# fritzsedlazeck/Sniffles

Measured on AMD Instinct MI355X. Metric: SV-signatures clustered/sec (clustering + calling + QC + genotype + INS consensus), higher is better.
Workload: dtype int32/f64

## Files before the change

### include/sniffles_amd.h

```cpp
#ifndef SNIFFLES_AMD_H
#define SNIFFLES_AMD_H

#include <stdint.h>

#ifdef __cplusplus
extern "C" {
#endif

#define SNF_ABI_VERSION 5

#define SNF_SVLEN_NONE INT32_MIN
#define SNF_SEQ_NONE (-1)
#define SNF_PS_NONE (-1)

enum snf_svtype {
  SNF_INS = 0, SNF_DEL = 1, SNF_DUP = 2, SNF_INV = 3, SNF_BND = 4,
  SNF_SINGLE_LEFT = 5, SNF_SINGLE_RIGHT = 6, SNF_NTYPES = 7
};

enum snf_source { SNF_SRC_INLINE = 0, SNF_SRC_SPLIT_PRIM = 1, SNF_SRC_SPLIT_SUP = 2, SNF_SRC_BND_SA = 3 };

enum snf_filter {
  SNF_F_PASS = 0, SNF_F_STDEV_POS, SNF_F_STDEV_LEN, SNF_F_SINGLE_BREAK, SNF_F_SVLEN_MIN,
  SNF_F_STRAND_BND, SNF_F_COV_CHANGE_DEL, SNF_F_COV_CHANGE_DUP, SNF_F_COV_CHANGE_INS,
// ... 219 lines not shown
struct snf_extract;
int snf_batch_add_task_device(snf_batch_t* b, struct snf_extract* x, const snf_task_input_t* meta);
int snf_batch_upload(snf_batch_t* b);
#define SNF_RUN_NONE 0
#define SNF_RUN_CANDIDATES 1
#define SNF_RUN_PASS 0x100
int snf_batch_open(const snf_config_t* cfg, int device, const snf_task_input_t* tasks, int32_t n_tasks, int run, snf_batch_t** out);
void snf_batch_destroy(snf_batch_t* b);

int snf_batch_call_candidates(snf_batch_t* b);

int snf_batch_finalize(snf_batch_t* b);

int snf_batch_pass(snf_batch_t* batch);

enum snf_output { SNF_OUT_CANDIDATES = 0, SNF_OUT_EXECUTE = 1, SNF_OUT_DEVICE = 2 };
int snf_batch_set_output(snf_batch_t* b, int mode);

int snf_batch_set_result_memory(snf_batch_t* b, void* block, int64_t block_bytes, void* alt, int64_t alt_bytes);

int snf_batch_fetch(snf_batch_t* b, int stage, snf_result_t* out);
int64_t snf_batch_n_candidates(snf_batch_t* b);

typedef struct snf_export_layout {
  int64_t n_calls, rnames_len, alt_pool_len;
  int64_t off_rnames, off_alt, bytes;
} snf_export_layout_t;
int snf_batch_export_device(snf_batch_t* b, void* dst_device, int64_t cap_bytes, snf_export_layout_t* layout);

int snf_batch_block_coverage(snf_batch_t* b, int32_t task_index, int32_t binsize, int64_t first_bin,
                             int64_t n_bins, int32_t* out);
// ... 418 lines not shown
```

### sniffles_amd/abi.py

```python
from __future__ import annotations

import ctypes as C
import math

import numpy as np

from .soa import LEAD_FIELDS, TaskInput

ABI_VERSION = 5

FILTERS = [
    "PASS", "STDEV_POS", "STDEV_LEN", "SINGLE_BREAK", "SVLEN_MIN", "STRAND_BND", "COV_CHANGE_DEL",
    "COV_CHANGE_DUP", "COV_CHANGE_INS", "INLINE_SA", "COV_VAR", "COV_CHANGE_FRAC_US", "COV_CHANGE_FRAC_SC",
    "COV_CHANGE_FRAC_CE", "COV_CHANGE_FRAC_ED", "SUPPORT_MIN", "GT_FAILED", "GT", "COV_MIN_GT", "ALN_NM",
    "MOSAIC_VAF", "SVLEN_MAX_MOSAIC", "STRAND", "STRAND_MOSAIC", "SVLEN_MIN_MOSAIC", "COV_MIN",
    "NOT_MOSAIC_VAF", "MOSAIC_SV_CLOSE_EDGE",
]
TASK_OK, TASK_ERR_UNBOUND_END = 0, 1

i32, i64, f64, u8p = C.c_int32, C.c_int64, C.c_double, C.POINTER(C.c_uint8)


class snf_config_t(C.Structure):
    _fields_ = [
# ... 72 lines not shown

class snf_result_t(C.Structure):
    _fields_ = [
        ("n_calls", i64), ("calls", C.POINTER(snf_call_t)),
        ("alt_pool_len", i64), ("alt_pool", u8p),
        ("rnames_len", i64), ("rnames", C.POINTER(C.c_uint32)),
        ("n_tasks", i64), ("task_status", C.POINTER(C.c_int32)),
        ("task_call_off", C.POINTER(C.c_int64)), ("coverage_average_total", C.POINTER(C.c_double)),
    ]


class snf_export_layout_t(C.Structure):
    _fields_ = [("n_calls", i64), ("rnames_len", i64), ("alt_pool_len", i64), ("off_rnames", i64), ("off_alt", i64), ("bytes", i64)]


OUT_CANDIDATES, OUT_EXECUTE, OUT_DEVICE = 0, 1, 2


class snf_clusters_t(C.Structure):
    _fields_ = [("n_clusters", i64)] + [(n, C.POINTER(C.c_int32)) for n in
                                        ("task_index", "svtype", "start", "end", "seed", "seed_index", "n_leads_long")] + \
               [("repeat", u8p), ("lead_off", C.POINTER(C.c_int64)), ("n_leads", i64), ("lead", C.POINTER(C.c_int32)),
                ("lead_svlen", C.POINTER(C.c_int32))]


class snf_combine_problem_t(C.Structure):
    _fields_ = [
        ("svtype", i32), ("n_cands", i32), ("n_groups", i32), ("n_sample_ids", i32),
        ("pos", C.POINTER(C.c_int32)), ("svlen", C.POINTER(C.c_int32)), ("support", C.POINTER(C.c_int32)),
        ("sample_id", C.POINTER(C.c_int32)), ("mate_contig", C.POINTER(C.c_int32)), ("mate_ref_start", C.POINTER(C.c_int32)),
        ("alt_off", C.POINTER(C.c_int64)), ("alt_pool", u8p),
# ... 425 lines not shown
```

### sniffles_amd/csrc/snf_lib.hip

```cpp
#include "snf_stage_final.h"
#include "snf_wave_refine.h"
#include "snf_wave_cons.h"
#include "snf_fused.h"
#include "snf_stage_window.h"
#include "snf_stage_out.h"
#include "snf_wave_call.h"
#include "snf_wave_call_g.h"
#include "snf_wave_refine_g.h"
#include "snf_ctx.h"
#include "snf_genotype.h"

#include <rocprim/device/device_radix_sort.hpp>
#include <rocprim/device/device_scan.hpp>

#include <fcntl.h>
#include <sys/file.h>
#include <unistd.h>

#include <atomic>
#include <map>
#include <tuple>
#include <cmath>
#include <ctime>
#include <memory>
// ... 228 lines not shown
  bool timing = true;
  bool time_all = false;
  int time_every = 8;
  bool time_now = true;
  uint64_t pass_count = 0;
  bool res_current = false;
  int64_t* h_rn_total = nullptr;
  int slots_d1w = 8192, slots_d2w = 8192, slots_e1w = 8192, slots_big = 8192;
  int read_key_bits = 64;
  std::vector<int32_t> h_rend_max;
  bool uploaded = false;
  bool finalized = false;
  int finalize_runs = 0;
  int rn_state = 0;
  int64_t pf_words = 0;
  struct PassGraph { hipGraph_t graph = nullptr; hipGraphExec_t exec = nullptr; int passes = 0; int rn_state = 0; int rn_defer = 0; size_t cap_out = 0, cap_alt = 0; };
  std::map<std::tuple<void*, void*, int>, PassGraph> graphs;
  int graph_mode = 0;
  bool in_flight = false;
  bool side_open = false;
  int slot_fd = -1;
  double pass_start_ms = 0.0;
  bool capturing = false;
  bool staged = false; bool staged_kernel = false, stage_block_copied = false, stage_alt_copied = false;
  bool graph_failed = false;
  int64_t h_n_big64 = 0;
  int64_t h_n_occ = 0; int win_cap = 0;
  bool reads_ready = false;
  bool cov_avg_ready = false;
  double gt_last_ms = 0;
  std::vector<snf_task_input_t> tasks;
// ... 7 lines not shown
  uint8_t* slab = nullptr; size_t slab_cap = 0, slab_used = 0, slab_next = (size_t)64 << 20;
  View v{};
  ReadPrep rp{};
  Counts* h_cnt = nullptr;
  void* sort_tmp[2] = {nullptr, nullptr}; size_t sort_tmp_bytes[2] = {0, 0};
  hipEvent_t ev_cls_fork = nullptr, ev_cls_join = nullptr;
  hipEvent_t ev_refined = nullptr, ev_fcopy = nullptr;
  bool fcopy_open = false;
  hipEvent_t ev_fork = nullptr, ev_join = nullptr, ev_fork3 = nullptr, ev_join3 = nullptr, ev_base = nullptr,
             ev_counts = nullptr, ev_rn = nullptr, ev_join4 = nullptr, ev_e3 = nullptr;
  int64_t tab_cap = 0, aln_cap = 0, cr_cap = 0, alt_cap = 0;
  HostBuf hb_calls, hb_rn, hb_res;
  bool pass_idle = false;
  HostBuf hb_out, hb_alt;
  std::vector<std::pair<void*, size_t>> ext_ranges;
  bool have_hist = false; int64_t hist_calls = 0, hist_small = 0, hist_large = 0, hist_copy = 0;
  bool have_big_hist = false; int64_t hist_big[3] = {0, 0, 0};
  bool skipped_big[3] = {false, false, false};
  int out_mode = 0;
  std::vector<int32_t> r_status; std::vector<int64_t> r_off; std::vector<double> r_cov;
  std::vector<int32_t> cl_task, cl_svtype, cl_start, cl_end, cl_seed, cl_seed_index, cl_nlong, cl_lead, cl_lead_svlen; std::vector<uint8_t> cl_repeat;
  std::vector<int64_t> cl_lead_off;
  std::vector<Timing> timings;
  std::vector<Timing> timing_acc;
  struct Ev { hipEvent_t a, b; const char* name; int64_t bytes; };
  std::vector<Ev> evs; size_t ev_used = 0;
};

template <class T>
T* dalloc_own(snf_batch_impl* b, size_t n) {
  size_t bytes = (n ? n : 1) * sizeof(T);
  void* p = nullptr;
  if (hipMalloc(&p, bytes) != hipSuccess) {
    (void)hipGetLastError();
    p = nullptr;
    g_slabs.trim(b->device);
    SNF_HIP(hipMalloc(&p, bytes));
  }
  b->bufs.push_back({p, bytes});
  return (T*)p;
}
template <class T>
// ... 986 lines not shown
  View& v = b->v;
  const int64_t N = v.NS;
  const dim3 grid(b->slots_d1w);
  const auto d1w = v.fuse_defer ? d1w_refine<true> : d1w_refine<false>;
  if (v.wave_path && b->k.d1_groups) {
    { ClassFork _f(b);
      KERNEL_GRID((v.fuse_defer ? d1g_refine<8, true> : d1g_refine<8, false>), grid, dim3(64), v, 0, "d1g_refine8", N * 36 / 3, heavy); }
    v.d1_from_list = 1;
    KERNEL_GRID(d1w, grid, dim3(64), v, 0, "d1w_refine", N * 36 - N * 36 / 3, heavy);
    v.d1_from_list = 0;
    join_classes(b);
  } else if (v.wave_path)
    KERNEL_GRID(d1w, grid, dim3(64), v, 0, "d1w_refine", N * 36, heavy);
  if (!(v.wave_path && b->fused)) KERNEL_N(d1_refine, v, N, v.wave_path ? 0 : N * 36, quiet);
  b->skipped_big[0] = b->skipped_big[1] = b->skipped_big[2] = false;
  if (v.wave_path && b->have_big_hist && b->hist_big[0] == 0) b->skipped_big[0] = true;
  else if (v.wave_path) KERNEL_GRID(x_big<0>, dim3(b->slots_big), dim3(64), v, 0, "x_big_refine", 0, heavy);
}
void enqueue_call(snf_batch_impl* b) {
  View& v = b->v;
  const int64_t N = v.NS;
  const bool ph = b->cfg.phase != 0;
  const dim3 grid(b->slots_d2w);
  const auto d2w = ph ? d2w_call<5, true> : d2w_call<5, false>;
  if (b->fused && v.chain_on) KERNEL_N(d1bc_rctable, v, N, 0, quiet);
  else if (b->fused) KERNEL_N(d1bk_rctable, v, N, 0, quiet);
  else {
    prim_exscan<uint32_t>(b, v.rcflag, v.rcscan, N + 1, "scan_refined");
    KERNEL_N(d1b_rctable, v, N, N * 4, quiet);
  }
  const bool call_forks = v.wave_path && b->k.d2_groups && classes_beside(b);
  if (v.fuse_defer && !call_forks) enqueue_fuse_copy(b, nullptr);
  if (v.wave_path && b->k.d2_groups) {
    { ClassFork _f(b);
      KERNEL_GRID((ph ? d2g_call<8, 4, true> : d2g_call<8, 4, false>), grid, dim3(64), v, 0, "d2g_call8", N * 32 / 3, heavy); }
    if (v.fuse_defer && call_forks) enqueue_fuse_copy(b, b->ev_cls_fork);
    const bool mid = b->k.d2_mid;
    if (mid) KERNEL_GRID((ph ? d2g_call<32, 4, true> : d2g_call<32, 4, false>), grid, dim3(64), v, 0, "d2g_call32", 0, heavy);
    v.d2_from_list = mid ? 2 : 1;
    KERNEL_GRID(d2w, grid, dim3(64), v, 0, "d2w_call", N * 32 - N * 32 / 3, heavy);
    v.d2_from_list = 0;
    join_classes(b);
  } else if (v.wave_path)
    KERNEL_GRID(d2w, grid, dim3(64), v, 0, "d2w_call", N * 32, heavy);
  if (!(v.wave_path && b->fused)) KERNEL_N(d2_call, v, N, v.wave_path ? 0 : N * 32, quiet);
  if (v.wave_path && b->have_big_hist && b->hist_big[1] == 0) b->skipped_big[1] = true;
  else if (v.wave_path) KERNEL_GRID(x_big<1>, dim3(b->slots_big), dim3(64), v, 0, "x_big_call", 0, heavy);
  if (b->fused && v.chain_on) KERNEL_N(d3cc_compact, v, N, 0, quiet);
  else if (b->fused) KERNEL_N(d3ck_compact, v, N, 0, quiet);
  else {
    prim_exscan<uint32_t>(b, v.cdflag, v.cdscan, N + 1, "scan_calls");
    KERNEL_N(d3_compact, v, N, 0, quiet);
  }
}
void enqueue_candidate_tail(snf_batch_impl* b) {
  View& v = b->v;
  const int64_t N = v.NS;
  KERNEL_N(d3_taskoff, v, tail_threads(v), 0, quiet);
  SNF_HIP(hipEventRecord(b->ev_counts, b->stream));
  fork_mark(b);
  if (b->fused) {
// ... 213 lines not shown
    const int stage_env = b->k.stage_out;
    const bool stage = !(v.out_mode & SNF_OUT_DEVICE) && !b->capturing && (stage_env == 1 || (stage_env < 0 && passes_overlap(b)));
    b->staged = stage; b->staged_kernel = stage && b->k.stage_copy_kernel;
    b->stage_block_copied = b->stage_alt_copied = false;
    const bool out_hbm = (v.out_mode & SNF_OUT_DEVICE) || stage;
    v.out_pin = out_hbm ? nullptr : (uint8_t*)b->hb_out.p;
    v.out_pin_cap = out_hbm ? 0 : (int64_t)b->hb_out.cap;
    v.stage_out_pin = b->staged_kernel ? (uint8_t*)b->hb_out.p : nullptr; v.stage_out_cap = b->staged_kernel ? (int64_t)b->hb_out.cap : 0;
    const size_t want_alt = (size_t)(v.pool_len / 8) + ((size_t)1 << 20);
    if (!(v.out_mode & SNF_OUT_DEVICE) && !b->hb_alt.external && b->hb_alt.cap < want_alt) b->hb_alt.ensure(want_alt);
    v.alt_pin = out_hbm ? nullptr : (uint8_t*)b->hb_alt.p;
    v.alt_pin_cap = out_hbm ? 0 : (int64_t)b->hb_alt.cap;
    v.stage_alt_pin = b->staged_kernel ? (uint8_t*)b->hb_alt.p : nullptr; v.stage_alt_cap = b->staged_kernel ? (int64_t)b->hb_alt.cap : 0;
  }
  v.out_valid = 1;
  int64_t n_calls_hint = b->hist_calls;
  if (!b->have_hist && NS > 0) {
    SNF_HIP(hipEventSynchronize(b->ev_counts));
    n_calls_hint = b->h_cnt->n_calls;
  }
  if (NS > 0) {
  {
    SideStream side(b);
    if (v.wave_path && b->finalize_runs++ > 0) dzero(b, v.big_cnt + 2 * 64 * 16, sizeof(uint32_t) * 64 * 16);
    if (v.wave_path) {
      int64_t grid = (n_calls_hint + v.e1_batch - 1) / v.e1_batch + 1;
      if (grid > (1 << 20)) grid = 1 << 20;
      KERNEL_GRID(e1w_finalize<5>, dim3((unsigned)grid), dim3(64), v, 0, "e1w_finalize", 0, heavy);
    }
    if (!v.wave_path) KERNEL_N(e1_finalize, v, NS, 0, quiet);
    if (v.wave_path && b->have_big_hist && b->hist_big[2] == 0 && b->finalize_runs == 1) b->skipped_big[2] = true;
    else if (v.wave_path) KERNEL_GRID(x_big<2>, dim3(b->slots_big), dim3(64), v, 0, "x_big_finalize", 0, heavy);
  }
  const bool fast_alt = v.wave_path && b->fused && NS <= ((int64_t)1 << 22) * 256;
  if (fast_alt)
  {
    const unsigned grid = (unsigned)((NS + 255) / 256);
    KERNEL_GRID(e2a_sizes, dim3(grid), dim3(256), v, 0, "e2a_sizes", 0, quiet);
    KERNEL_GRID(e3b_offsets, dim3(grid), dim3(256), v, 0, "e3b_offsets", 0, quiet);
    SNF_HIP(hipEventRecord(b->ev_e3, b->stream));
    {
      SideStream side(b);
      SNF_HIP(hipStreamWaitEvent(b->stream2, b->ev_e3, 0));
      SNF_HIP(hipStreamWaitEvent(b->stream2, b->ev_rn, 0));
      enqueue_output_head(b);
      stage_copy_block(b);
    }
    if (!b->have_hist) {
      d2h(b, b->h_cnt, v.cnt, sizeof(Counts));
      dsync(b);
      const Counts& c = *b->h_cnt;
      b->hist_small = (int64_t)c.n_cls[1]; b->hist_large = (int64_t)(c.n_cls[2] + c.n_cls[3] + c.n_cls[4] + c.n_cls[5]); b->hist_copy = (int64_t)c.n_cls[0];
      b->hist_calls = c.n_calls; b->have_hist = true;
    }
    join_fuse_copy(b);
    enqueue_consensus_wave(b, b->hist_small + 1, b->hist_large + 1, b->hist_copy + 1);
    stage_copy_alt(b);
    join_side(b);
    join_fourth(b);
  }
  else
  {
    d2h(b, b->h_cnt, v.cnt, sizeof(Counts));
    dsync(b);
    const int64_t nc = b->h_cnt->n_calls;
    dzero(b, v.stripes, sizeof(unsigned long long) * 4 * 64 * 16);
    KERNEL_N(e2_best, v, nc + 1, 0, heavy);
    prim_exscan<uint32_t>(b, v.fN, v.pN, nc + 1, "scan_alt");
    prim_exscan<uint32_t>(b, v.fL, v.pL, nc + 1, "scan_cons");
    prim_exscan<int64_t>(b, v.sz_tab, v.sc_tab, nc + 1, "scan_cons_sizes");
    prim_exscan<int64_t>(b, v.sz_aln, v.sc_aln, nc + 1, "scan_cons_sizes");
// ... 11 lines not shown
    join_fourth(b);
    enqueue_output_head(b);
  }
  } else {
    join_side(b);
    join_fourth(b);
    enqueue_output_head(b);
  }
  KERNEL_N(z1_results, v, tail_threads(v), 0, quiet);
  b->res_current = true;
}

bool pass_graph_ok(snf_batch_impl* b) {
  const View& v = b->v;
  if (b->graph_mode == 1 && pacing_of(b).passes_in_flight.load() > 1) return false;
  return b->graph_mode && !b->graph_failed && b->have_hist && b->fused && v.front && v.wave_path && !b->k.timeline && !b->time_all &&
         v.NS > 0 && !b->k.readprep_each_pass && !b->k.serial;
}
void run_pass(snf_batch_impl* b) {
  View& v = b->v;
  pass_begins(b);
  join_open_candidates(b);
  if (!pass_graph_ok(b)) { run_call_candidates(b); run_finalize(b); return; }
  const auto key = std::make_tuple((void*)b->hb_out.p, (void*)b->hb_alt.p, v.out_mode);
  auto& g = b->graphs[key];
  if (g.exec && (g.cap_out != b->hb_out.cap || g.cap_alt != b->hb_alt.cap)) {
    (void)hipGraphExecDestroy(g.exec); (void)hipGraphDestroy(g.graph); g = snf_batch_impl::PassGraph{};
  }
  g.passes++;
  const bool sampled = b->timing && (b->time_all || b->time_every == 1 || (b->time_every > 1 && b->pass_count % (uint64_t)b->time_every == 0));
  if (g.exec && !sampled) {
    b->pass_idle = false;
    reset_timing(b); b->pass_count++;
    SNF_HIP(hipGraphLaunch(g.exec, b->stream));
    b->reads_ready = true; b->cov_avg_ready = true; b->finalized = true; b->finalize_runs = 1; b->res_current = true;
    b->rn_state = g.rn_state; v.rn_defer = g.rn_defer; v.out_valid = 1;
    return;
  }
  if (g.exec || g.passes < 2) { run_call_candidates(b); run_finalize(b); return; }
  const bool tm = b->timing;
  b->timing = false;
  hipGraph_t graph = nullptr;
  bool ok = hipStreamBeginCapture(b->stream, hipStreamCaptureModeThreadLocal) == hipSuccess;
  if (ok) {
    b->capturing = true;
    const uint64_t count_before = b->pass_count;
    try { run_call_candidates(b); run_finalize(b); }
    catch (const std::exception& e) {
      (void)hipStreamEndCapture(b->stream, &graph); if (graph) (void)hipGraphDestroy(graph); graph = nullptr; ok = false; (void)hipGetLastError();
      b->pass_count = count_before;
      if (v.prof) fprintf(stderr, "[SNF_PROF] pass graph: capture gave up (%s); the pass runs eagerly\n", e.what());
// ... 5 lines not shown
    b->capturing = false;
    if (ok) ok = hipStreamEndCapture(b->stream, &graph) == hipSuccess && graph != nullptr;
  }
  b->timing = tm;
  hipGraphExec_t exec = nullptr;
  if (ok) ok = hipGraphInstantiate(&exec, graph, nullptr, nullptr, 0) == hipSuccess && exec != nullptr;
  if (!ok) {
    (void)hipGetLastError();
    if (graph) (void)hipGraphDestroy(graph);
    b->graph_failed = true;
    if (v.prof) fprintf(stderr, "[SNF_PROF] pass graph: capture failed, passes stay eager\n");
    run_call_candidates(b); run_finalize(b);
    return;
  }
  g.graph = graph; g.exec = exec; g.rn_state = b->rn_state; g.rn_defer = v.rn_defer; g.cap_out = b->hb_out.cap; g.cap_alt = b->hb_alt.cap;
  if (v.prof) { size_t nn = 0; (void)hipGraphGetNodes(graph, nullptr, &nn); fprintf(stderr, "[SNF_PROF] pass graph: captured (%zu nodes)\n", nn); }
  SNF_HIP(hipGraphLaunch(g.exec, b->stream));
}
void destroy_graphs(snf_batch_impl* b) {
  for (auto& kv : b->graphs) { if (kv.second.exec) (void)hipGraphExecDestroy(kv.second.exec); if (kv.second.graph) (void)hipGraphDestroy(kv.second.graph); }
  b->graphs.clear();
}

void collect_timings(snf_batch_impl* b) {
  b->timings.clear();
#ifdef SNF_ITRACE
  if (b->k.prof && b->v.itrace) {
    static const char* nm[SNF_IT_SLOTS] = {"w1_hist", "w3_scatter", "w4s_segment", "w6t_emit", "d1g_refine", "d1w_refine", "d2g_call", "d2w_call", "e3b_offsets",
                                           "e1w_finalize", "cons SMALL", "cons LARGE", "d4s_coverage", "f4w_emit", "cons ROWS", ""};
    std::vector<uint32_t> h((size_t)SNF_IT_SLOTS * SNF_IT_CAP * 2);
// ... 119 lines not shown

void do_fetch(snf_batch_impl* b, int stage, snf_result_t* out) {
  SNF_TRACE(stage >= 1 ? "snf_batch_fetch(1): wait + result block" : "snf_batch_fetch(0): wait + candidates");
  View& v = b->v;
  int T = v.T;
  b->r_status.assign(T, 0); b->r_off.assign(T + 1, 0); b->r_cov.assign(T, NAN);
  full_sync(b);
  pass_waited(b);
  if (b->h_cnt->overflow) fail(b->h_cnt->overflow & 2 ? "internal: hand-over list of the call kernels overflowed" : "internal: fused-sequence pool overflow");
  if (v.prof) {
    const Counts& c = *b->h_cnt;
    fprintf(stderr, "[SNF_PROF] counts: valid %lld windows %lld bins %lld seeds %lld clusters %lld refined %lld calls %lld | cons calls %lld reads %lld "
                    "fallback %lld alt bytes %lld fused bytes through the shared counter %llu (the rest in the waves' own slices; the split depends on scheduling, the total and the capacity do not) | ALT lists copy %llu small %llu large %llu/%llu/%llu/%llu thread %llu rows %llu\n", (long long)c.n_valid, (long long)c.n_occ, (long long)c.n_bins, (long long)c.n_seeds, (long long)c.n_clusters,
            (long long)c.n_rc, (long long)c.n_calls, (long long)c.n_cons, (long long)c.n_cons_reads, (long long)c.n_cons_fallback,
            (long long)c.alt_total, c.pool_extra_used, c.n_cls[0], c.n_cls[1], c.n_cls[2], c.n_cls[3], c.n_cls[4], c.n_cls[5], c.n_cls[6], c.n_cls[7]);
    fprintf(stderr, "[SNF_PROF] merge scan: %lld runs, %lld groups redone serially (run_gap %d)\n", (long long)c.n_runs, (long long)c.n_dirty_groups, (int)v.run_gap);
  }
  memcpy(b->r_status.data(), v.res_status, (size_t)T * sizeof(int32_t));
  memcpy(b->r_cov.data(), v.res_cov, (size_t)T * sizeof(double));
  if (stage >= 1 && b->finalized) {
    const bool alt_late = settle_alt_stage(b);
    {
      const Counts& c = *b->h_cnt;
      bool skipped_work = false;
      for (int k = 0; k < 3; k++) {
        if (b->skipped_big[k] && c.n_big[k] > 0) skipped_work = true;
        b->hist_big[k] = c.n_big[k];
      }
      if (skipped_work) { b->pass_idle = true; fail("internal: a pass skipped x_big although items were handed to it (the handle's next pass launches it)"); }
      b->have_big_hist = true;
      b->hist_small = (int64_t)c.n_cls[1]; b->hist_large = (int64_t)(c.n_cls[2] + c.n_cls[3] + c.n_cls[4] + c.n_cls[5]); b->hist_copy = (int64_t)c.n_cls[0];
      b->hist_calls = c.n_calls; b->have_hist = true;
    }
    const OutHdr h = *v.res_out;
    const uint8_t* base = (const uint8_t*)b->hb_out.p;
    const int64_t alt_total_now = b->h_cnt->alt_total;
    const bool block_there = !h.in_pinned && b->staged_kernel && b->stage_block_copied && v.stage_out_pin == (uint8_t*)b->hb_out.p && h.bytes <= v.stage_out_cap;
    const bool alt_there = !b->h_cnt->alt_in_pinned && b->staged_kernel && b->stage_alt_copied && !alt_late && v.stage_alt_pin == (uint8_t*)b->hb_alt.p && alt_total_now <= v.stage_alt_cap;
    bool need_sync = false;
    std::unique_lock<std::mutex> copy_turn(pacing_of(b).copy_mu, std::defer_lock);
    if (b->staged && pace_copy_turn() && ((!h.in_pinned && !block_there) || (!b->h_cnt->alt_in_pinned && !alt_there))) copy_turn.lock();
    if (!h.in_pinned && !block_there) {
      v.out_pin = nullptr; v.out_pin_cap = 0;
      base = (const uint8_t*)b->hb_out.ensure((size_t)h.bytes + 256);
      d2h_timed(b, (void*)base, v.out_dev, (size_t)h.bytes, "d2h_block");
      need_sync = true;
    }
// ... 597 lines not shown
}

int snf_batch_upload(snf_batch_t* bb) {
  SNF_TRY({
    auto b = reinterpret_cast<snf_batch_impl*>(bb);
    if (!b) fail("null batch");
    if (b->uploaded) fail("batch already uploaded");
    SNF_HIP(hipSetDevice(b->device));
    do_upload(b);
  })
}

int snf_batch_open(const snf_config_t* cfg, int device, const snf_task_input_t* tasks, int32_t n_tasks, int run, snf_batch_t** out) {
  if (out) *out = nullptr;
  if (!out || (n_tasks > 0 && !tasks) || n_tasks < 0) { g_err = "snf_batch_open: null argument"; return 1; }
  if (run != SNF_RUN_NONE && run != SNF_RUN_CANDIDATES && !((run & SNF_RUN_PASS) && (run & ~SNF_RUN_PASS) <= (SNF_OUT_EXECUTE | SNF_OUT_DEVICE))) {
    g_err = "snf_batch_open: unknown run mode"; return 1;
  }
  snf_batch_t* h = nullptr;
  int rc = snf_batch_create(cfg, device, &h);
  for (int32_t t = 0; rc == 0 && t < n_tasks; t++) rc = snf_batch_add_task(h, &tasks[t]);
  if (rc == 0) rc = snf_batch_upload(h);
  if (rc == 0 && run == SNF_RUN_CANDIDATES) rc = snf_batch_call_candidates(h);
  if (rc == 0 && (run & SNF_RUN_PASS)) { rc = snf_batch_set_output(h, run & ~SNF_RUN_PASS); if (rc == 0) rc = snf_batch_pass(h); }
  if (rc != 0) { const std::string keep = g_err; if (h) snf_batch_destroy(h); g_err = keep; return rc; }
  *out = h;
  return 0;
}

void snf_batch_destroy(snf_batch_t* bb) {
  auto b = reinterpret_cast<snf_batch_impl*>(bb);
// ... 23 lines not shown
  for (auto& e : b->ext_ranges) (void)hipHostUnregister(e.first);
  b->ext_ranges.clear();
  if (b->stream) g_streams.give(b->device, b->stream);
  if (b->stream2) g_streams.give(b->device, b->stream2);
  if (b->stream3) g_streams.give(b->device, b->stream3);
  if (b->stream4) g_streams.give(b->device, b->stream4);
  if (b->ev_join4) (void)hipEventDestroy(b->ev_join4);
  delete b;
}

int snf_batch_call_candidates(snf_batch_t* bb) {
  SNF_TRY({
    auto b = reinterpret_cast<snf_batch_impl*>(bb);
    if (!b || !b->uploaded) fail("batch not uploaded");
    SNF_HIP(hipSetDevice(b->device));
    run_call_candidates(b);
  })
}

int snf_batch_pass(snf_batch_t* bb) {
  SNF_TRY({
    auto b = reinterpret_cast<snf_batch_impl*>(bb);
    if (!b || !b->uploaded) fail("batch not uploaded");
    SNF_HIP(hipSetDevice(b->device));
    run_pass(b);
  })
}

int snf_batch_finalize(snf_batch_t* bb) {
  SNF_TRY({
// ... 31 lines not shown
  if (!b || !b->uploaded || !b->h_cnt) return -1;
  return b->v.NS > 0 ? b->h_cnt->n_calls : 0;
}

int64_t snf_trim_caches(int device) {
  int64_t bytes = (int64_t)g_slabs.trim(device);
  bytes += (int64_t)g_pinned.trim();
  (void)g_streams.trim(device);
  return bytes;
}

int snf_batch_set_output(snf_batch_t* bb, int mode) {
  SNF_TRY({
    auto b = reinterpret_cast<snf_batch_impl*>(bb);
    if (!b) fail("null batch");
    if (mode < 0 || mode > (SNF_OUT_EXECUTE | SNF_OUT_DEVICE)) fail("unknown output mode");
    b->out_mode = mode; b->v.out_mode = mode;
  })
}

int snf_batch_set_result_memory(snf_batch_t* bb, void* block, int64_t block_bytes, void* alt, int64_t alt_bytes) {
  SNF_TRY({
    auto b = reinterpret_cast<snf_batch_impl*>(bb);
    if (!b) fail("null batch");
    if ((block == nullptr) != (alt == nullptr) || block_bytes < 0 || alt_bytes < 0) fail("snf_batch_set_result_memory: both sections or none");
    SNF_HIP(hipSetDevice(b->device));
    if (b->uploaded && !b->pass_idle) full_sync(b);
    if (!block) { b->hb_out.release(); b->hb_alt.release(); }
    else { b->hb_out.adopt(block, (size_t)block_bytes, b->ext_ranges); b->hb_alt.adopt(alt, (size_t)alt_bytes, b->ext_ranges); }
  })
}
// ... 119 lines not shown
```

### sniffles_amd/csrc/snf_stage_cluster.h

```cpp
#pragma once
#include "snf_exact.h"
#include "snf_view.h"

namespace snf {

#define SNF_KEY_INVALID (~0ull)
SNF_HD int key_grp(uint64_t key) { return (int)(key >> 32); }
SNF_HD int grp_svtype(int g) { return g & 7; }
SNF_HD int grp_task(int g) { return g >> 3; }

SNF_HD bool lead_is_long(const View& v, uint32_t o) {
  return v.in_svtype[o] == SNF_INS && v.in_svlen[o] == SNF_SVLEN_NONE;
}

SNF_HD int64_t pf_cell(const View& v, int t, int svtype, uint64_t bin) {
  const int64_t c0 = v.t_cell_off[t], nb = (v.t_cell_off[t + 1] - c0) / SNF_NTYPES;
  return c0 + (int64_t)svtype * nb + (int64_t)bin;
}
SNF_HD void a1_keys_body(int64_t i, const View& v) {
  int t = v.lead_task[i];
  int64_t rs = v.in_ref_start[i];
  bool valid = rs >= 0 && rs < v.t_contig_len[t];
  uint64_t bin = valid ? (uint64_t)(rs / v.cfg.cluster_binsize) : 0;
  const int svtype = v.in_svtype[i];
// ... 73 lines not shown
}

SNF_HD void a4_binstats_body(int64_t b, const View& v) {
  if (b >= v.cnt->n_bins) { v.eligflag[b] = 0; return; }
  int32_t lo = v.bin_lo[b], hi = v.bin_lo[b + 1];
  int n_normal = 0;
  uint32_t hc[3] = {0, 0, 0};
  for (int32_t p = lo; p < hi; p++) {
    uint32_t o = v.val_out[p];
    if (p - lo + 1 > v.cfg.consensus_max_reads_bin) v.seqnull[o] = 1;
    uint8_t h = v.in_hap[o];
    if (hc[h] < 65535u) hc[h]++;
    if (!lead_is_long(v, o)) n_normal++;
  }
  for (int h = 0; h < 3; h++) v.bin_hap[3 * b + h] = (uint16_t)hc[h];
  bool el = n_normal >= v.cfg.dev_min_leads_cluster;
  v.bin_elig[b] = el;
  v.eligflag[b] = el ? 1u : 0u;
  int g = key_grp(v.bin_key[b]);
  if (b == 0 || key_grp(v.bin_key[b - 1]) != g) v.grp_first_bin[g] = (int32_t)b;
}

SNF_HD void a5_leadflags_body(int64_t p, const View& v) {
  uint32_t fn = 0, fl = 0;
  if (p < v.cnt->n_valid) {
    uint32_t b = v.headscan[p + 1] - 1;
    if (v.bin_elig[b]) {
      if (lead_is_long(v, v.val_out[p])) fl = 1; else fn = 1;
    }
  }
  v.fN[p] = fn;
  v.fL[p] = fl;
  if (p == 0) { v.fN[v.NS] = 0; v.fL[v.NS] = 0; v.eligflag[v.NS] = 0; }
}
// ... 327 lines not shown
```

### sniffles_amd/csrc/snf_stage_window.h

```cpp
#pragma once
#include "snf_fused.h"
#include "snf_wave_refine.h"

namespace snf {

#define SNF_WIN_MAXCAP 1024

SNF_HD uint32_t win_pack(const View& v, uint32_t bin_low, bool is_long, uint32_t hap) { return bin_low | ((is_long ? 1u : 0u) << 12) | (hap << 13); }
SNF_HD uint32_t win_bin_low(uint32_t a) { return a & 0xfffu; }
SNF_HD bool win_is_long(uint32_t a) { return (a >> 12) & 1u; }
SNF_HD uint32_t win_hap(uint32_t a) { return (a >> 13) & 3u; }
SNF_D bool win_of_lead(const View& v, int64_t i, uint32_t* w, uint32_t* attr) {
  const int t = v.lead_task[i];
  const int64_t rs = v.in_ref_start[i];
  if (rs < 0 || rs >= v.t_contig_len[t]) return false;
  const uint64_t bin = (uint64_t)(rs / v.cfg.cluster_binsize);
  const int svtype = v.in_svtype[i];
  const int64_t w0 = v.t_win_off[t], nwin = (v.t_win_off[t + 1] - w0) / SNF_NTYPES;
  *w = (uint32_t)(w0 + (int64_t)svtype * nwin + (int64_t)(bin >> v.win_bits));
  *attr = win_pack(v, (uint32_t)(bin & ((1u << v.win_bits) - 1u)), svtype == SNF_INS && v.in_svlen[i] == SNF_SVLEN_NONE, v.in_hap[i]);
  return true;
}

SNF_D int win_group(bool valid, uint32_t w, int* count, bool* leader) {
// ... 138 lines not shown
    if (i >= (int64_t)v.cnt->n_w4big) return;
    i = v.w4_list[i];
  }
  const int64_t B0 = 64 * i;
  const int64_t n_valid = v.win_ready ? v.win_n_valid : v.cnt->n_valid;
  uint64_t w0 = 0;
  if (B0 + lane < n_valid) w0 = v.key_in[B0 + lane];
  uint32_t k0 = 0, k1 = 0;
  if (B0 < n_valid) { k0 = v.blk_k0[i]; k1 = B0 + 64 <= n_valid ? v.blk_k0[i + 1] : (uint32_t)(v.win_ready ? v.win_n_occ : v.cnt->n_occ); }
  const int nw = (int)(k1 - k0);
  if (nw <= 0) { if (lane == 0) { v.ws_seeds[i] = 0; v.ws_nf[i] = 0; v.ws_nl[i] = 0; } return; }
  uint4 wr = make_uint4(0, 0, 0, 0);
  if (lane < nw) wr = ((const uint4*)v.wlist)[k0 + lane];
  const int xlo = (int)((int64_t)(uint32_t)__builtin_amdgcn_readfirstlane((int)wr.z) - B0);
  const int xhi = (int)((int64_t)(uint32_t)__builtin_amdgcn_readlane((int)(wr.z + wr.y), nw - 1) - B0);
  if (v.w4_mode == 1 && __shfl(wave_incl_max(lane < nw ? (int)wr.y : 0), 63, 64) > CAP) {
    if (lane == 0) v.w4_list[atomicAdd(&v.cnt->n_w4big, 1ull)] = (int32_t)i;
    return;
  }
  uint64_t wd[E];
  wd[0] = w0;
#pragma unroll
  for (int j = 1; j < E; j++) { const int x = lane + 64 * j; wd[j] = x < xhi ? v.key_in[B0 + x] : 0ull; }
  if (lane < nw) {
    const int t = (int)wr.w;
    const int64_t o0 = v.t_win_off[t], nwin = (v.t_win_off[t + 1] - o0) / SNF_NTYPES, rem = (int64_t)wr.x - o0;
    wS[lane] = (uint32_t)((int64_t)wr.z - B0); wG[lane] = (uint32_t)(t * 8 + (int)(rem / nwin)); wB[lane] = (uint32_t)((rem % nwin) << v.win_bits);
  }
#pragma unroll
  for (int j = 0; j < E; j++) { const int x = lane + 64 * j; if (x < xhi) { sA[x] = 0; sB[x] = 0; widx[x] = 0; } }
  const int nall = __shfl(wave_incl_max(lane < nw ? (int)wr.y : 0), 63, 64);
  for (int p = lane; p < nall + PAD; p += 64) keys[xhi + p] = ~0ull;
  __syncthreads();
  if (lane < nw) widx[wS[lane]] = (uint16_t)(lane + 1);
  __syncthreads();
  uint64_t e[E];
  {
    int carry = 0;
#pragma unroll
    for (int j = 0; j < E; j++) {
      e[j] = 0;
      if (64 * j < xhi) {
        const int x = lane + 64 * j;
// ... 62 lines not shown
  }
  __syncthreads();
  int cs = 0, cf = 0, cl = 0;
  const unsigned long long below = (1ull << lane) - 1ull;
#pragma unroll
  for (int j = 0; j < E; j++) {
    const int x = lane + 64 * j;
    if (64 * j >= xhi) break;
    const bool own = x >= xlo && x < xhi;
    bool f_seed = false, f_norm = false, f_long = false, f_null = false;
    int h = 0, all = 0, with_len = 0;
    if (own) {
      h = hpos[x];
      const uint32_t A = sA[h];
      all = (int)(A & 0xffffu); with_len = (int)(A >> 16);
      const bool elig = with_len >= v.cfg.dev_min_leads_cluster;
      f_norm = elig && !wkey_long(sk[j]); f_long = elig && wkey_long(sk[j]); f_seed = elig && x == h;
      f_null = x - h + 1 > v.cfg.consensus_max_reads_bin;
    }
    const unsigned long long bn = __ballot(f_norm), bl = __ballot(f_long), bs = __ballot(f_seed);
    const uint32_t rn = (uint32_t)(cf + __popcll(bn & below)), rl = (uint32_t)(cl + __popcll(bl & below)), rs = (uint32_t)(cs + __popcll(bs & below));
    if (own) {
      const uint32_t hi = (f_norm ? SNF_WS_NORM : 0u) | (f_long ? SNF_WS_LONG : 0u) | (f_null ? SNF_WS_SEQNULL : 0u) | (f_seed ? SNF_WS_SEED : 0u) |
                          ((f_norm ? rn : rl) << 4) | ((uint32_t)j << 16) | (f_seed ? rs << 21 : 0u);
      v.key_out[B0 + x] = ((uint64_t)hi << 32) | (uint64_t)wkey_index(sk[j]);
      if (f_seed) {
        const uint32_t B = sB[h];
        const int wl = (int)wkey_widx(sk[j]);
        const int64_t start = ((int64_t)wB[wl] + (int64_t)wkey_bin(sk[j])) * v.cfg.cluster_binsize;
        v.whead[B0 + x] = (uint64_t)with_len | ((uint64_t)all << 16) | ((uint64_t)(B & 0xffffu) << 32) | ((uint64_t)(B >> 16) << 48);
        v.whead2[B0 + x] = (uint64_t)(uint32_t)(int32_t)start | ((uint64_t)wG[wl] << 32) | ((uint64_t)(f_norm ? rl : rn) << 52);
// ... 81 lines not shown
```

### sniffles_amd/csrc/snf_view.h

```cpp
#pragma once
#include "../../include/sniffles_amd.h"
#include "snf_rt.h"

namespace snf {

struct Counts {
  int64_t n_valid, n_bins, n_seeds, NF, NLL, n_runs, n_clusters, n_rc, n_calls;
  int64_t n_ins_calls, alt_total, n_cons, tab_total, aln_total, n_cons_reads, rn_total;
  int64_t n_dirty_groups;
  int64_t n_kept;
  int64_t n_big[3];
  int64_t n_occ;
  int64_t max_win;
  int64_t n_big64;
  unsigned long long n_w4big;
  int64_t n_cons_fallback;
  unsigned long long cons_bytes[4];
  unsigned long long n_cls[8];
  unsigned long long pool_extra_used;
#ifdef SNF_CONS_PROFILE
  unsigned long long dbg[32];
#endif
#ifdef SNF_C1_PROFILE
  unsigned long long c1p[16];
#endif
  int32_t overflow;
  int32_t alt_in_pinned;
};

struct GtEntry {
// ... 109 lines not shown
  uint32_t* rflag;

  const int32_t *nm_start, *nm_end;
  const int64_t* t_nm_off;
  const int32_t* t_cov_exact;

  const int32_t* tr_start; const int32_t* tr_end; const int32_t* tr_pmax;

  int32_t prefilter;
  uint32_t* pf_bm;
  const int64_t* t_cell_off;
  uint64_t* pf_key;
  uint32_t *pf_keep, *pf_scan;
  int32_t front;
  int32_t win_bits;
  int64_t NW;
  const int64_t* t_win_off;
  int32_t win_ready;
  int32_t win_stats;
  int64_t win_n_valid, win_n_occ;
  uint32_t *wcnt, *wfill;
  uint32_t* wbase;
  uint32_t* wlist;
  uint32_t* blk_k0;
  uint32_t *ws_seeds, *ws_nf, *ws_nl;
  uint64_t* whead;
  uint64_t* whead2;
  uint64_t *key_in, *key_out; uint32_t *val_in, *val_out;
  int key32, key_bin_bits, key_nbits;
  uint32_t *headflag, *headscan;
// ... 81 lines not shown
  int32_t* cls_list[8];
  uint32_t* big_cnt;
  int32_t* big_list;
  int64_t big_cap;
  int32_t big_wave;
  int32_t e1_batch;
  int32_t* w4_list; int32_t w4_mode, _pad_w4;
  int32_t heavy_n;
  int32_t wave_uniform;
  int32_t* w7;
  const LeadRec* stage_R; int32_t* stage_w; int32_t stage_cap; int32_t _pad_stage;
  uint8_t* aln_kept_w;
  int64_t* crl_off; int32_t* crl_len;
};

#define SNF_IT_SLOTS 16
#define SNF_IT_CAP (1 << 17)
#ifdef SNF_ITRACE
struct ItScope {
  uint32_t* o; unsigned long long t0;
  __device__ ItScope(const View& v, int slot) : o(nullptr), t0(wall_clock64()) {
    if (v.itrace && threadIdx.x == 0 && blockIdx.x < (unsigned)SNF_IT_CAP) o = v.itrace + 2 * ((int64_t)slot * SNF_IT_CAP + blockIdx.x);
  }
  __device__ ~ItScope() { if (o) { o[0] = (uint32_t)t0; o[1] = (uint32_t)(wall_clock64() - t0) | 0x80000000u; } }
};
#define IT_SCOPE(slot) ItScope it_scope_(v, slot);
#else
#define IT_SCOPE(slot)
#endif

// ... 2 lines not shown
```

### sniffles_amd/parallel.py

```python
from __future__ import annotations

import os

from . import lib, sv
from .abi import TASK_ERR_UNBOUND_END

LAZY_CALLS = os.environ.get("SNF_EAGER_CALLS") != "1"


class Task:
    def __init__(self, id, sv_id, contig, start, end, config, assigned_process_id=None, lead_provider=None,
                 tandem_repeats=None, regions=None, device: int = 0):
        self.id, self.sv_id, self.contig, self.start, self.end = id, sv_id, contig, start, end
        self.config = config
        self.assigned_process_id = assigned_process_id
        self.lead_provider = lead_provider
        self.tandem_repeats = tandem_repeats
        self.regions = regions
        self.device = device
        self.coverage_average_total = None
        self._batch = None
        self._ti = None
        self._prep = None
        self._lazy = None
        self._served = False

    def prepare(self, config, execute=None):
        from .abi import OUT_CANDIDATES, OUT_EXECUTE
        if self._prep is not None or self._server() is not None:
            return
        self._release()
        self._ti = self._task_input(config)
        from .soa import DeviceTaskInput
        if isinstance(self._ti, DeviceTaskInput):
            return
        run = lib.Batch.RUN_CANDIDATES if execute is None else (lib.Batch.RUN_PASS | (OUT_EXECUTE if execute else OUT_CANDIDATES))
        self._prep = {"mode": execute, "pending": lib.Batch.open_in_background(config, [self._ti], device=self.device, run=run)}

    def _prepared(self, execute) -> bool:
        box, self._prep = self._prep, None
        if box is None:
            return False
        if box["mode"] != execute:
            box["pending"].discard()
            return False
        self._batch = box["pending"].result()
        self._adopt()
        return True

    def _task_input(self, config):
        lp = self.lead_provider
# ... 93 lines not shown
                                       keep_all=bool(config.no_qc or getattr(config, "snf", None) is not None))
            out = self._lazy.make()
        else:
            out = sv.materialize_candidates(res, self._ti, 0, len(res.calls), svcall_cls, bnd_cls, sv.SVCallPostprocessingInfo, self._batch)
        self.sv_id += len(out)
        self.coverage_average_total = float(res.coverage_average_total[0])
        return out

    def _drop_lazy(self):
        src = getattr(self, "_lazy", None)
        self._lazy = None
        if src is not None:
            src.detach()

    def call_records(self, config, execute: bool = False):
        from .abi import OUT_CANDIDATES, OUT_EXECUTE
        if not self._prepared(bool(execute)):
            self._open(config)
            self._batch.set_output(OUT_EXECUTE if execute else OUT_CANDIDATES)
            self._batch.run_pass()
        res = self._batch.fetch(1, copy=False)
        if int(res.task_status[0]) == TASK_ERR_UNBOUND_END:
            raise UnboundLocalError("local variable 'end' referenced before assignment")
        self._finalized = True
        self.sv_id += int(self._batch.n_candidates())
        self.coverage_average_total = float(res.coverage_average_total[0])
        return res, self._ti

    def finalize_candidates(self, candidates, keep_qc_fails, config) -> list:
        import numpy as np
        if getattr(self, "_served", False):
            if getattr(self, "_finalized", False):
                raise RuntimeError("finalize_candidates needs the candidates of this task's call_candidates")
            candidates = list(candidates)
# ... 345 lines not shown
```

Measured before the change: 3.776 billion.

## Skip single-breakend seeds and windows in execute passes when QC drops them

```diff
diff --git a/include/sniffles_amd.h b/include/sniffles_amd.h
--- a/include/sniffles_amd.h
+++ b/include/sniffles_amd.h
@@ -257,7 +257,7 @@
 
 int snf_batch_pass(snf_batch_t* batch);
 
-enum snf_output { SNF_OUT_CANDIDATES = 0, SNF_OUT_EXECUTE = 1, SNF_OUT_DEVICE = 2 };
+enum snf_output { SNF_OUT_CANDIDATES = 0, SNF_OUT_EXECUTE = 1, SNF_OUT_DEVICE = 2, SNF_OUT_ALL_CANDIDATES = 4 };
 int snf_batch_set_output(snf_batch_t* b, int mode);
 
 int snf_batch_set_result_memory(snf_batch_t* b, void* block, int64_t block_bytes, void* alt, int64_t alt_bytes);
diff --git a/sniffles_amd/abi.py b/sniffles_amd/abi.py
--- a/sniffles_amd/abi.py
+++ b/sniffles_amd/abi.py
@@ -110,7 +110,7 @@
     _fields_ = [("n_calls", i64), ("rnames_len", i64), ("alt_pool_len", i64), ("off_rnames", i64), ("off_alt", i64), ("bytes", i64)]
 
 
-OUT_CANDIDATES, OUT_EXECUTE, OUT_DEVICE = 0, 1, 2
+OUT_CANDIDATES, OUT_EXECUTE, OUT_DEVICE, OUT_ALL_CANDIDATES = 0, 1, 2, 4
 
 
 class snf_clusters_t(C.Structure):
diff --git a/sniffles_amd/csrc/snf_lib.hip b/sniffles_amd/csrc/snf_lib.hip
--- a/sniffles_amd/csrc/snf_lib.hip
+++ b/sniffles_amd/csrc/snf_lib.hip
@@ -266,7 +266,8 @@
   int finalize_runs = 0;
   int rn_state = 0;
   int64_t pf_words = 0;
-  struct PassGraph { hipGraph_t graph = nullptr; hipGraphExec_t exec = nullptr; int passes = 0; int rn_state = 0; int rn_defer = 0; size_t cap_out = 0, cap_alt = 0; };
+  struct PassGraph { hipGraph_t graph = nullptr; hipGraphExec_t exec = nullptr; int passes = 0; int rn_state = 0; int rn_defer = 0; size_t cap_out = 0, cap_alt = 0;
+                     bool skipped_big[3] = {false, false, false}; };
   std::map<std::tuple<void*, void*, int>, PassGraph> graphs;
   int graph_mode = 0;
   bool in_flight = false;
@@ -304,8 +305,10 @@
   bool pass_idle = false;
   HostBuf hb_out, hb_alt;
   std::vector<std::pair<void*, size_t>> ext_ranges;
-  bool have_hist = false; int64_t hist_calls = 0, hist_small = 0, hist_large = 0, hist_copy = 0;
-  bool have_big_hist = false; int64_t hist_big[3] = {0, 0, 0};
+  struct PassHints {
+    bool have_hist = false; int64_t hist_calls = 0, hist_small = 0, hist_large = 0, hist_copy = 0;
+    bool have_big_hist = false; int64_t hist_big[3] = {0, 0, 0};
+  } hints[2];
   bool skipped_big[3] = {false, false, false};
   int out_mode = 0;
   std::vector<int32_t> r_status; std::vector<int64_t> r_off; std::vector<double> r_cov;
@@ -316,6 +319,7 @@
   struct Ev { hipEvent_t a, b; const char* name; int64_t bytes; };
   std::vector<Ev> evs; size_t ev_used = 0;
 };
+inline snf_batch_impl::PassHints& hints_of(snf_batch_impl* b) { return b->hints[b->v.skip_single ? 1 : 0]; }
 
 template <class T>
 T* dalloc_own(snf_batch_impl* b, size_t n) {
@@ -1332,7 +1336,7 @@
     KERNEL_GRID(d1w, grid, dim3(64), v, 0, "d1w_refine", N * 36, heavy);
   if (!(v.wave_path && b->fused)) KERNEL_N(d1_refine, v, N, v.wave_path ? 0 : N * 36, quiet);
   b->skipped_big[0] = b->skipped_big[1] = b->skipped_big[2] = false;
-  if (v.wave_path && b->have_big_hist && b->hist_big[0] == 0) b->skipped_big[0] = true;
+  if (v.wave_path && hints_of(b).have_big_hist && hints_of(b).hist_big[0] == 0) b->skipped_big[0] = true;
   else if (v.wave_path) KERNEL_GRID(x_big<0>, dim3(b->slots_big), dim3(64), v, 0, "x_big_refine", 0, heavy);
 }
 void enqueue_call(snf_batch_impl* b) {
@@ -1362,7 +1366,7 @@
   } else if (v.wave_path)
     KERNEL_GRID(d2w, grid, dim3(64), v, 0, "d2w_call", N * 32, heavy);
   if (!(v.wave_path && b->fused)) KERNEL_N(d2_call, v, N, v.wave_path ? 0 : N * 32, quiet);
-  if (v.wave_path && b->have_big_hist && b->hist_big[1] == 0) b->skipped_big[1] = true;
+  if (v.wave_path && hints_of(b).have_big_hist && hints_of(b).hist_big[1] == 0) b->skipped_big[1] = true;
   else if (v.wave_path) KERNEL_GRID(x_big<1>, dim3(b->slots_big), dim3(64), v, 0, "x_big_call", 0, heavy);
   if (b->fused && v.chain_on) KERNEL_N(d3cc_compact, v, N, 0, quiet);
   else if (b->fused) KERNEL_N(d3ck_compact, v, N, 0, quiet);
@@ -1606,8 +1610,8 @@
     v.stage_alt_pin = b->staged_kernel ? (uint8_t*)b->hb_alt.p : nullptr; v.stage_alt_cap = b->staged_kernel ? (int64_t)b->hb_alt.cap : 0;
   }
   v.out_valid = 1;
-  int64_t n_calls_hint = b->hist_calls;
-  if (!b->have_hist && NS > 0) {
+  int64_t n_calls_hint = hints_of(b).hist_calls;
+  if (!hints_of(b).have_hist && NS > 0) {
     SNF_HIP(hipEventSynchronize(b->ev_counts));
     n_calls_hint = b->h_cnt->n_calls;
   }
@@ -1621,7 +1625,7 @@
       KERNEL_GRID(e1w_finalize<5>, dim3((unsigned)grid), dim3(64), v, 0, "e1w_finalize", 0, heavy);
     }
     if (!v.wave_path) KERNEL_N(e1_finalize, v, NS, 0, quiet);
-    if (v.wave_path && b->have_big_hist && b->hist_big[2] == 0 && b->finalize_runs == 1) b->skipped_big[2] = true;
+    if (v.wave_path && hints_of(b).have_big_hist && hints_of(b).hist_big[2] == 0 && b->finalize_runs == 1) b->skipped_big[2] = true;
     else if (v.wave_path) KERNEL_GRID(x_big<2>, dim3(b->slots_big), dim3(64), v, 0, "x_big_finalize", 0, heavy);
   }
   const bool fast_alt = v.wave_path && b->fused && NS <= ((int64_t)1 << 22) * 256;
@@ -1638,15 +1642,15 @@
       enqueue_output_head(b);
       stage_copy_block(b);
     }
-    if (!b->have_hist) {
+    if (!hints_of(b).have_hist) {
       d2h(b, b->h_cnt, v.cnt, sizeof(Counts));
       dsync(b);
       const Counts& c = *b->h_cnt;
-      b->hist_small = (int64_t)c.n_cls[1]; b->hist_large = (int64_t)(c.n_cls[2] + c.n_cls[3] + c.n_cls[4] + c.n_cls[5]); b->hist_copy = (int64_t)c.n_cls[0];
-      b->hist_calls = c.n_calls; b->have_hist = true;
+      hints_of(b).hist_small = (int64_t)c.n_cls[1]; hints_of(b).hist_large = (int64_t)(c.n_cls[2] + c.n_cls[3] + c.n_cls[4] + c.n_cls[5]); hints_of(b).hist_copy = (int64_t)c.n_cls[0];
+      hints_of(b).hist_calls = c.n_calls; hints_of(b).have_hist = true;
     }
     join_fuse_copy(b);
-    enqueue_consensus_wave(b, b->hist_small + 1, b->hist_large + 1, b->hist_copy + 1);
+    enqueue_consensus_wave(b, hints_of(b).hist_small + 1, hints_of(b).hist_large + 1, hints_of(b).hist_copy + 1);
     stage_copy_alt(b);
     join_side(b);
     join_fourth(b);
@@ -1688,11 +1692,15 @@
 bool pass_graph_ok(snf_batch_impl* b) {
   const View& v = b->v;
   if (b->graph_mode == 1 && pacing_of(b).passes_in_flight.load() > 1) return false;
-  return b->graph_mode && !b->graph_failed && b->have_hist && b->fused && v.front && v.wave_path && !b->k.timeline && !b->time_all &&
+  return b->graph_mode && !b->graph_failed && hints_of(b).have_hist && b->fused && v.front && v.wave_path && !b->k.timeline && !b->time_all &&
          v.NS > 0 && !b->k.readprep_each_pass && !b->k.serial;
+}
+bool pass_skips_single(const snf_batch_impl* b) {
+  return (b->v.out_mode & SNF_OUT_EXECUTE) && !(b->v.out_mode & SNF_OUT_ALL_CANDIDATES) && !b->cfg.no_qc && !b->cfg.dev_output_candidates;
 }
 void run_pass(snf_batch_impl* b) {
   View& v = b->v;
+  v.skip_single = pass_skips_single(b) ? 1 : 0;
   pass_begins(b);
   join_open_candidates(b);
   if (!pass_graph_ok(b)) { run_call_candidates(b); run_finalize(b); return; }
@@ -1709,6 +1717,7 @@
     SNF_HIP(hipGraphLaunch(g.exec, b->stream));
     b->reads_ready = true; b->cov_avg_ready = true; b->finalized = true; b->finalize_runs = 1; b->res_current = true;
     b->rn_state = g.rn_state; v.rn_defer = g.rn_defer; v.out_valid = 1;
+    for (int k = 0; k < 3; k++) b->skipped_big[k] = g.skipped_big[k];
     return;
   }
   if (g.exec || g.passes < 2) { run_call_candidates(b); run_finalize(b); return; }
@@ -1744,6 +1753,7 @@
     return;
   }
   g.graph = graph; g.exec = exec; g.rn_state = b->rn_state; g.rn_defer = v.rn_defer; g.cap_out = b->hb_out.cap; g.cap_alt = b->hb_alt.cap;
+  for (int k = 0; k < 3; k++) g.skipped_big[k] = b->skipped_big[k];
   if (v.prof) { size_t nn = 0; (void)hipGraphGetNodes(graph, nullptr, &nn); fprintf(stderr, "[SNF_PROF] pass graph: captured (%zu nodes)\n", nn); }
   SNF_HIP(hipGraphLaunch(g.exec, b->stream));
 }
@@ -1893,6 +1903,8 @@
                     "fallback %lld alt bytes %lld fused bytes through the shared counter %llu (the rest in the waves' own slices; the split depends on scheduling, the total and the capacity do not) | ALT lists copy %llu small %llu large %llu/%llu/%llu/%llu thread %llu rows %llu\n", (long long)c.n_valid, (long long)c.n_occ, (long long)c.n_bins, (long long)c.n_seeds, (long long)c.n_clusters,
             (long long)c.n_rc, (long long)c.n_calls, (long long)c.n_cons, (long long)c.n_cons_reads, (long long)c.n_cons_fallback,
             (long long)c.alt_total, c.pool_extra_used, c.n_cls[0], c.n_cls[1], c.n_cls[2], c.n_cls[3], c.n_cls[4], c.n_cls[5], c.n_cls[6], c.n_cls[7]);
+    if (v.skip_single) fprintf(stderr, "[SNF_PROF] skip single: %llu of %lld waves of w4s_segment left early (every window of theirs a single-breakend one)\n",
+                               c.n_w4left, (long long)((v.N + 63) / 64));
     fprintf(stderr, "[SNF_PROF] merge scan: %lld runs, %lld groups redone serially (run_gap %d)\n", (long long)c.n_runs, (long long)c.n_dirty_groups, (int)v.run_gap);
   }
   memcpy(b->r_status.data(), v.res_status, (size_t)T * sizeof(int32_t));
@@ -1904,12 +1916,12 @@
       bool skipped_work = false;
       for (int k = 0; k < 3; k++) {
         if (b->skipped_big[k] && c.n_big[k] > 0) skipped_work = true;
-        b->hist_big[k] = c.n_big[k];
+        hints_of(b).hist_big[k] = c.n_big[k];
       }
       if (skipped_work) { b->pass_idle = true; fail("internal: a pass skipped x_big although items were handed to it (the handle's next pass launches it)"); }
-      b->have_big_hist = true;
-      b->hist_small = (int64_t)c.n_cls[1]; b->hist_large = (int64_t)(c.n_cls[2] + c.n_cls[3] + c.n_cls[4] + c.n_cls[5]); b->hist_copy = (int64_t)c.n_cls[0];
-      b->hist_calls = c.n_calls; b->have_hist = true;
+      hints_of(b).have_big_hist = true;
+      hints_of(b).hist_small = (int64_t)c.n_cls[1]; hints_of(b).hist_large = (int64_t)(c.n_cls[2] + c.n_cls[3] + c.n_cls[4] + c.n_cls[5]); hints_of(b).hist_copy = (int64_t)c.n_cls[0];
+      hints_of(b).hist_calls = c.n_calls; hints_of(b).have_hist = true;
     }
     const OutHdr h = *v.res_out;
     const uint8_t* base = (const uint8_t*)b->hb_out.p;
@@ -2537,7 +2549,7 @@
 int snf_batch_open(const snf_config_t* cfg, int device, const snf_task_input_t* tasks, int32_t n_tasks, int run, snf_batch_t** out) {
   if (out) *out = nullptr;
   if (!out || (n_tasks > 0 && !tasks) || n_tasks < 0) { g_err = "snf_batch_open: null argument"; return 1; }
-  if (run != SNF_RUN_NONE && run != SNF_RUN_CANDIDATES && !((run & SNF_RUN_PASS) && (run & ~SNF_RUN_PASS) <= (SNF_OUT_EXECUTE | SNF_OUT_DEVICE))) {
+  if (run != SNF_RUN_NONE && run != SNF_RUN_CANDIDATES && !((run & SNF_RUN_PASS) && (run & ~SNF_RUN_PASS) <= (SNF_OUT_EXECUTE | SNF_OUT_DEVICE | SNF_OUT_ALL_CANDIDATES))) {
     g_err = "snf_batch_open: unknown run mode"; return 1;
   }
   snf_batch_t* h = nullptr;
@@ -2591,6 +2603,7 @@
     auto b = reinterpret_cast<snf_batch_impl*>(bb);
     if (!b || !b->uploaded) fail("batch not uploaded");
     SNF_HIP(hipSetDevice(b->device));
+    b->v.skip_single = 0;
     run_call_candidates(b);
   })
 }
@@ -2652,7 +2665,7 @@
   SNF_TRY({
     auto b = reinterpret_cast<snf_batch_impl*>(bb);
     if (!b) fail("null batch");
-    if (mode < 0 || mode > (SNF_OUT_EXECUTE | SNF_OUT_DEVICE)) fail("unknown output mode");
+    if (mode < 0 || mode > (SNF_OUT_EXECUTE | SNF_OUT_DEVICE | SNF_OUT_ALL_CANDIDATES)) fail("unknown output mode");
     b->out_mode = mode; b->v.out_mode = mode;
   })
 }
diff --git a/sniffles_amd/csrc/snf_stage_cluster.h b/sniffles_amd/csrc/snf_stage_cluster.h
--- a/sniffles_amd/csrc/snf_stage_cluster.h
+++ b/sniffles_amd/csrc/snf_stage_cluster.h
@@ -111,10 +111,10 @@
     if (!lead_is_long(v, o)) n_normal++;
   }
   for (int h = 0; h < 3; h++) v.bin_hap[3 * b + h] = (uint16_t)hc[h];
-  bool el = n_normal >= v.cfg.dev_min_leads_cluster;
+  int g = key_grp(v.bin_key[b]);
+  bool el = n_normal >= v.cfg.dev_min_leads_cluster && !seed_type_skipped(v, g & 7);
   v.bin_elig[b] = el;
   v.eligflag[b] = el ? 1u : 0u;
-  int g = key_grp(v.bin_key[b]);
   if (b == 0 || key_grp(v.bin_key[b - 1]) != g) v.grp_first_bin[g] = (int32_t)b;
 }
 
diff --git a/sniffles_amd/csrc/snf_stage_window.h b/sniffles_amd/csrc/snf_stage_window.h
--- a/sniffles_amd/csrc/snf_stage_window.h
+++ b/sniffles_amd/csrc/snf_stage_window.h
@@ -176,6 +176,20 @@
   if (lane < nw) wr = ((const uint4*)v.wlist)[k0 + lane];
   const int xlo = (int)((int64_t)(uint32_t)__builtin_amdgcn_readfirstlane((int)wr.z) - B0);
   const int xhi = (int)((int64_t)(uint32_t)__builtin_amdgcn_readlane((int)(wr.z + wr.y), nw - 1) - B0);
+  uint32_t wgrp = 0, wbin0 = 0;
+  if (lane < nw) {
+    const int t = (int)wr.w;
+    const int64_t o0 = v.t_win_off[t], nwin = (v.t_win_off[t + 1] - o0) / SNF_NTYPES, rem = (int64_t)wr.x - o0;
+    wgrp = (uint32_t)(t * 8 + (int)(rem / nwin)); wbin0 = (uint32_t)((rem % nwin) << v.win_bits);
+  }
+  if (v.skip_single && !__ballot(lane < nw && !seed_type_skipped(v, (int)(wgrp & 7u)))) {
+    for (int x = lane; x < xhi; x += 64) if (x >= xlo) v.key_out[B0 + x] = 0;
+    if (lane == 0) {
+      v.ws_seeds[i] = 0; v.ws_nf[i] = 0; v.ws_nl[i] = 0;
+      if (v.prof) atomicAdd(&v.cnt->n_w4left, 1ull);
+    }
+    return;
+  }
   if (v.w4_mode == 1 && __shfl(wave_incl_max(lane < nw ? (int)wr.y : 0), 63, 64) > CAP) {
     if (lane == 0) v.w4_list[atomicAdd(&v.cnt->n_w4big, 1ull)] = (int32_t)i;
     return;
@@ -184,11 +198,7 @@
   wd[0] = w0;
 #pragma unroll
   for (int j = 1; j < E; j++) { const int x = lane + 64 * j; wd[j] = x < xhi ? v.key_in[B0 + x] : 0ull; }
-  if (lane < nw) {
-    const int t = (int)wr.w;
-    const int64_t o0 = v.t_win_off[t], nwin = (v.t_win_off[t + 1] - o0) / SNF_NTYPES, rem = (int64_t)wr.x - o0;
-    wS[lane] = (uint32_t)((int64_t)wr.z - B0); wG[lane] = (uint32_t)(t * 8 + (int)(rem / nwin)); wB[lane] = (uint32_t)((rem % nwin) << v.win_bits);
-  }
+  if (lane < nw) { wS[lane] = (uint32_t)((int64_t)wr.z - B0); wG[lane] = wgrp; wB[lane] = wbin0; }
 #pragma unroll
   for (int j = 0; j < E; j++) { const int x = lane + 64 * j; if (x < xhi) { sA[x] = 0; sB[x] = 0; widx[x] = 0; } }
   const int nall = __shfl(wave_incl_max(lane < nw ? (int)wr.y : 0), 63, 64);
@@ -281,7 +291,7 @@
       h = hpos[x];
       const uint32_t A = sA[h];
       all = (int)(A & 0xffffu); with_len = (int)(A >> 16);
-      const bool elig = with_len >= v.cfg.dev_min_leads_cluster;
+      const bool elig = with_len >= v.cfg.dev_min_leads_cluster && !(v.skip_single && seed_type_skipped(v, (int)(wG[wkey_widx(sk[j])] & 7u)));
       f_norm = elig && !wkey_long(sk[j]); f_long = elig && wkey_long(sk[j]); f_seed = elig && x == h;
       f_null = x - h + 1 > v.cfg.consensus_max_reads_bin;
     }
diff --git a/sniffles_amd/csrc/snf_view.h b/sniffles_amd/csrc/snf_view.h
--- a/sniffles_amd/csrc/snf_view.h
+++ b/sniffles_amd/csrc/snf_view.h
@@ -14,6 +14,7 @@
   int64_t max_win;
   int64_t n_big64;
   unsigned long long n_w4big;
+  unsigned long long n_w4left;
   int64_t n_cons_fallback;
   unsigned long long cons_bytes[4];
   unsigned long long n_cls[8];
@@ -153,6 +154,7 @@
   uint32_t *pf_keep, *pf_scan;
   int32_t front;
   int32_t win_bits;
+  int32_t skip_single, _pad_ss;
   int64_t NW;
   const int64_t* t_win_off;
   int32_t win_ready;
@@ -264,6 +266,8 @@
   int64_t* crl_off; int32_t* crl_len;
 };
 
+SNF_HD bool seed_type_skipped(const View& v, int svtype) { return v.skip_single && svtype >= SNF_SINGLE_LEFT; }
+
 #define SNF_IT_SLOTS 16
 #define SNF_IT_CAP (1 << 17)
 #ifdef SNF_ITRACE
diff --git a/sniffles_amd/parallel.py b/sniffles_amd/parallel.py
--- a/sniffles_amd/parallel.py
+++ b/sniffles_amd/parallel.py
@@ -26,7 +26,7 @@
         self._served = False
 
     def prepare(self, config, execute=None):
-        from .abi import OUT_CANDIDATES, OUT_EXECUTE
+        from .abi import OUT_ALL_CANDIDATES, OUT_CANDIDATES, OUT_EXECUTE
         if self._prep is not None or self._server() is not None:
             return
         self._release()
@@ -34,7 +34,7 @@
         from .soa import DeviceTaskInput
         if isinstance(self._ti, DeviceTaskInput):
             return
-        run = lib.Batch.RUN_CANDIDATES if execute is None else (lib.Batch.RUN_PASS | (OUT_EXECUTE if execute else OUT_CANDIDATES))
+        run = lib.Batch.RUN_CANDIDATES if execute is None else (lib.Batch.RUN_PASS | (OUT_EXECUTE | OUT_ALL_CANDIDATES if execute else OUT_CANDIDATES))
         self._prep = {"mode": execute, "pending": lib.Batch.open_in_background(config, [self._ti], device=self.device, run=run)}
 
     def _prepared(self, execute) -> bool:
@@ -158,10 +158,10 @@
             src.detach()
 
     def call_records(self, config, execute: bool = False):
-        from .abi import OUT_CANDIDATES, OUT_EXECUTE
+        from .abi import OUT_ALL_CANDIDATES, OUT_CANDIDATES, OUT_EXECUTE
         if not self._prepared(bool(execute)):
             self._open(config)
-            self._batch.set_output(OUT_EXECUTE if execute else OUT_CANDIDATES)
+            self._batch.set_output(OUT_EXECUTE | OUT_ALL_CANDIDATES if execute else OUT_CANDIDATES)
             self._batch.run_pass()
         res = self._batch.fetch(1, copy=False)
         if int(res.task_status[0]) == TASK_ERR_UNBOUND_END:
```

Measured after the change: 4.042 billion (median of 6 runs). +7.0%, better.
